# cmhungsteve/TA3N

Hardware: AMD Instinct MI355X
Metric: src+tgt videos/sec per train step, UCF->HMDB_full 5-seg TA3N (higher is better)
Workload: dtype bf16

## Files before the change

### ta3n_amd/csrc/ta3n_gemm_kernel.h

```cpp
#pragma once
#include <hip/hip_runtime.h>
#include <cstdlib>
#include <cstring>

#include <type_traits>

#include "ta3n_kernels.h"

using namespace ta3n;

namespace {

typedef float f32x16 __attribute__((ext_vector_type(16)));
typedef __attribute__((address_space(3))) void lds_void_t;

constexpr int BKC = 64;

__device__ __forceinline__ float4 zero4() { return make_float4(0.f, 0.f, 0.f, 0.f); }

__device__ __forceinline__ void glds16(const float *gsrc, unsigned lds_byte_addr) {
    unsigned keep;
    lds_byte_addr = __builtin_amdgcn_readfirstlane(lds_byte_addr);
    asm volatile("s_mov_b32 %0, m0\n\ts_mov_b32 m0, %2\n\ts_nop 0\n\tglobal_load_lds_dwordx4 %1, off\n\ts_mov_b32 m0, %0"
                 : "=&s"(keep) : "v"(gsrc), "s"(lds_byte_addr) : "memory");
// ... 434 lines not shown
                    unsigned ah[4], al[4], bh[4], bl[4];
#pragma unroll
                    for (int h = 0; h < 2; ++h)
#pragma unroll
                        for (int e = 0; e < 2; ++e) {
                            ah[2 * h + e] = hi2(av[q + h][2 * e], av[q + h][2 * e + 1]);
                            al[2 * h + e] = lo2(av[q + h][2 * e], av[q + h][2 * e + 1], ah[2 * h + e]);
                            bh[2 * h + e] = hi2(bv[q + h][2 * e], bv[q + h][2 * e + 1]);
                            bl[2 * h + e] = lo2(bv[q + h][2 * e], bv[q + h][2 * e + 1], bh[2 * h + e]);
                        }
                    const u32x4 AH = {ah[0], ah[1], ah[2], ah[3]}, AL = {al[0], al[1], al[2], al[3]};
                    const u32x4 BH = {bh[0], bh[1], bh[2], bh[3]}, BL = {bl[0], bl[1], bl[2], bl[3]};
                    acc = __builtin_amdgcn_mfma_f32_32x32x16_bf16(__builtin_bit_cast(bf16x8, AL), __builtin_bit_cast(bf16x8, BH), acc, 0, 0, 0);
                    acc = __builtin_amdgcn_mfma_f32_32x32x16_bf16(__builtin_bit_cast(bf16x8, AH), __builtin_bit_cast(bf16x8, BL), acc, 0, 0, 0);
                    acc = __builtin_amdgcn_mfma_f32_32x32x16_bf16(__builtin_bit_cast(bf16x8, AH), __builtin_bit_cast(bf16x8, BH), acc, 0, 0, 0);
                }
            }
        } else {
#pragma unroll
            for (int q = 0; q < NQ; ++q) {
                if (FULL || 4 * (wk * GPW + 2 * q) < krem) {
                    unsigned ah[2], al[2], bh[2], bl[2];
#pragma unroll
                    for (int e = 0; e < 2; ++e) {
                        ah[e] = hi2(av[q][2 * e], av[q][2 * e + 1]); al[e] = lo2(av[q][2 * e], av[q][2 * e + 1], ah[e]);
                        bh[e] = hi2(bv[q][2 * e], bv[q][2 * e + 1]); bl[e] = lo2(bv[q][2 * e], bv[q][2 * e + 1], bh[e]);
                    }
                    const u32x2 AH = {ah[0], ah[1]}, AL = {al[0], al[1]}, BH = {bh[0], bh[1]}, BL = {bl[0], bl[1]};
                    acc = __builtin_amdgcn_mfma_f32_32x32x8bf16_1k(__builtin_bit_cast(s16x4, AL), __builtin_bit_cast(s16x4, BH), acc, 0, 0, 0);
                    acc = __builtin_amdgcn_mfma_f32_32x32x8bf16_1k(__builtin_bit_cast(s16x4, AH), __builtin_bit_cast(s16x4, BL), acc, 0, 0, 0);
                    acc = __builtin_amdgcn_mfma_f32_32x32x8bf16_1k(__builtin_bit_cast(s16x4, AH), __builtin_bit_cast(s16x4, BH), acc, 0, 0, 0);
                }
            }
        }
        return;
    }
    if (BF) {
        if (NQ % 2 == 0) {
#pragma unroll
            for (int q = 0; q < NQ; q += 2) {
                if (FULL || 4 * (wk * GPW + 2 * q) < krem) {
                    const u32x4 a = {pack_bf16(av[q][0], av[q][1]), pack_bf16(av[q][2], av[q][3]),
                                     pack_bf16(av[q + 1][0], av[q + 1][1]), pack_bf16(av[q + 1][2], av[q + 1][3])};
                    const u32x4 b = {pack_bf16(bv[q][0], bv[q][1]), pack_bf16(bv[q][2], bv[q][3]),
                                     pack_bf16(bv[q + 1][0], bv[q + 1][1]), pack_bf16(bv[q + 1][2], bv[q + 1][3])};
                    acc = __builtin_amdgcn_mfma_f32_32x32x16_bf16(__builtin_bit_cast(bf16x8, a), __builtin_bit_cast(bf16x8, b),
                                                                  acc, 0, 0, 0);
                }
            }
        } else {
#pragma unroll
            for (int q = 0; q < NQ; ++q) {
                if (FULL || 4 * (wk * GPW + 2 * q) < krem) {
                    const u32x2 a = {pack_bf16(av[q][0], av[q][1]), pack_bf16(av[q][2], av[q][3])};
                    const u32x2 b = {pack_bf16(bv[q][0], bv[q][1]), pack_bf16(bv[q][2], bv[q][3])};
                    acc = __builtin_amdgcn_mfma_f32_32x32x8bf16_1k(__builtin_bit_cast(s16x4, a), __builtin_bit_cast(s16x4, b), acc,
                                                                   0, 0, 0);
                }
            }
        }
        return;
    }
#pragma unroll
    for (int q = 0; q < NQ; ++q) {
        if (FULL || 4 * (wk * GPW + 2 * q) < krem) {
#pragma unroll
            for (int j = 0; j < 4; ++j) acc = __builtin_amdgcn_mfma_f32_32x32x2f32(av[q][j], bv[q][j], acc, 0, 0, 0);
        }
    }
}

__device__ __forceinline__ void st_pub(float *p, f32x4 v) { asm volatile("global_store_dwordx4 %0, %1, off sc0 sc1" ::"v"(p), "v"(v) : "memory"); }
__device__ __forceinline__ void st_pub(void *p, u32x2 v) { asm volatile("global_store_dwordx2 %0, %1, off sc0 sc1" ::"v"(p), "v"(v) : "memory"); }
__device__ __forceinline__ void st_pub(float *p, float v) { asm volatile("global_store_dword %0, %1, off sc0 sc1" ::"v"(p), "v"(v) : "memory"); }
__device__ __forceinline__ void st_pub(unsigned short *p, unsigned v) { asm volatile("global_store_short %0, %1, off sc0 sc1" ::"v"(p), "v"(v) : "memory"); }

__device__ __forceinline__ void store_twin4(unsigned short *tp, unsigned w0, unsigned w1, int nrem, bool vec, bool pub) {
    if (nrem >= 4 && vec) {
        if (pub) st_pub(tp, u32x2{w0, w1});
        else *reinterpret_cast<u32x2 *>(tp) = u32x2{w0, w1};
    } else {
        const unsigned short h[4] = {(unsigned short)(w0 & 0xFFFF), (unsigned short)(w0 >> 16), (unsigned short)(w1 & 0xFFFF), (unsigned short)(w1 >> 16)};
#pragma unroll
        for (int e = 0; e < 4; ++e)
            if (e < nrem) { if (pub) st_pub(tp + e, (unsigned)h[e]); else tp[e] = h[e]; }
    }
}

constexpr int CHAIN_SPIN_LIMIT = 1 << 20;
__device__ __forceinline__ void chain_wait(const Task &t, const Wait *__restrict__ waits, int *__restrict__ cnt, int tid, int knobs) {
    const int nwait = (knobs & 1024) ? 0 : t.wait_count;
    if (nwait > 0) {
        if (tid < 64) {
            for (int w0 = 0; w0 < nwait; w0 += 64) {
                const bool mine = w0 + tid < nwait;
                Wait w{0, 0};
                if (mine) w = waits[t.wait_begin + w0 + tid];
                bool ok = !mine;
                int spins = 0;
                for (;;) {
                    if (!ok) ok = ((knobs & 2048) ? __hip_atomic_fetch_add(cnt + 2 + w.counter, 0, __ATOMIC_RELAXED, __HIP_MEMORY_SCOPE_AGENT)
                                                  : __hip_atomic_load(cnt + 2 + w.counter, __ATOMIC_RELAXED, __HIP_MEMORY_SCOPE_AGENT)) >= w.target;
                    if (__all(ok)) break;
                    if (++spins > CHAIN_SPIN_LIMIT) {
                        if (tid == 0) __hip_atomic_store(cnt + 1, 1 + (int)blockIdx.x, __ATOMIC_RELAXED, __HIP_MEMORY_SCOPE_AGENT);
                        break;
                    }
                    if ((spins & 1023) == 0 && __hip_atomic_load(cnt + 1, __ATOMIC_RELAXED, __HIP_MEMORY_SCOPE_AGENT) != 0) break;
                    for (int z = 0; z < (knobs & 255); ++z) __builtin_amdgcn_s_sleep(8);
                }
            }
            if (!(knobs & 256)) __builtin_amdgcn_fence(__ATOMIC_ACQUIRE, "agent");
        }
        __syncthreads();
    }
}
__device__ __forceinline__ void chain_exit(int sig, int *__restrict__ cnt, int n_counters, int tid, int knobs) {
    if ((knobs & 512) && sig < 0) return;
    asm volatile("s_waitcnt vmcnt(0)" ::: "memory");
    __syncthreads();
    if (tid == 0) {
        if (knobs & 512) { __hip_atomic_fetch_add(cnt + 2 + sig, 1, __ATOMIC_RELAXED, __HIP_MEMORY_SCOPE_AGENT); return; }
        if (sig >= 0) {
            const int before = __hip_atomic_fetch_add(cnt + 2 + sig, 1, __ATOMIC_RELAXED, __HIP_MEMORY_SCOPE_AGENT);
            asm volatile("s_waitcnt vmcnt(0)" ::"v"(before) : "memory");
        }
        const int done = __hip_atomic_fetch_add(cnt, 1, __ATOMIC_RELAXED, __HIP_MEMORY_SCOPE_AGENT);
        if (done == (int)gridDim.x - 1) {
            for (int i = 0; i < n_counters; ++i) __hip_atomic_store(cnt + 2 + i, 0, __ATOMIC_RELAXED, __HIP_MEMORY_SCOPE_AGENT);
            __hip_atomic_store(cnt, 0, __ATOMIC_RELAXED, __HIP_MEMORY_SCOPE_AGENT);
        }
    }
}

__device__ __forceinline__ const float *base_ptr(const Ptrs &p, int base) {
    switch (base) {
        case BASE_X: return p.x;
        case BASE_P: return p.p;
        case BASE_G: return p.g;
        case BASE_P16: return p.p16;
        default: return p.ws;
    }
}

}

#ifdef TA3N_GEMM_STAMPS
#define TA3N_STAMP_SLOTS 16
#define TA3N_STAMP_FLOATS (8192 * TA3N_STAMP_SLOTS * 2)
#define GSTAMP_PTR (reinterpret_cast<unsigned long long *>(const_cast<float *>(ptrs.ws) + zeros_off - TA3N_STAMP_FLOATS))
#define GSTAMP(i) do { if (threadIdx.x == 0 && blockIdx.x < 8192) GSTAMP_PTR[blockIdx.x * TA3N_STAMP_SLOTS + (i)] = __builtin_amdgcn_s_memtime(); } while (0)
#define GSTAMP_VAL(i, v) do { if (threadIdx.x == 0 && blockIdx.x < 8192) GSTAMP_PTR[blockIdx.x * TA3N_STAMP_SLOTS + (i)] = (unsigned long long)(v); } while (0)
#define GSTAMP_W1(i, v) do { if (threadIdx.x == 64 && blockIdx.x < 8192) GSTAMP_PTR[blockIdx.x * TA3N_STAMP_SLOTS + (i)] = (unsigned long long)(v); } while (0)
#define KSTAMP_DECL unsigned long long ks_wait = 0, ks_comp = 0, ks_t = 0; int ks_n = 0
#define KSTAMP_BEGIN_WAIT do { ks_t = __builtin_amdgcn_s_memtime(); } while (0)
#define KSTAMP_END_WAIT do { const unsigned long long n_ = __builtin_amdgcn_s_memtime(); ks_wait += n_ - ks_t; ks_t = n_; ++ks_n; } while (0)
#define KSTAMP_END_COMP do { if (ks_t != 0) { const unsigned long long n_ = __builtin_amdgcn_s_memtime(); ks_comp += n_ - ks_t; } } while (0)
#else
#define GSTAMP(i) do { } while (0)
#define GSTAMP_VAL(i, v) do { } while (0)
#define KSTAMP_DECL do { } while (0)
#define KSTAMP_BEGIN_WAIT do { } while (0)
#define KSTAMP_END_WAIT do { } while (0)
#define KSTAMP_END_COMP do { } while (0)
#endif

namespace ta3n {

template <int WM, int WN, int WK, int BF, int NS, int RM, int RN, int KV = 63>
__device__ __forceinline__ void gemm_tile(const Task &t, const Seg *__restrict__ segs, const Ptrs &ptrs, int hyper_off, int zeros_off,
                                          int twin_off, const SgdSide &side, int pair_delta, int knobs) {
    constexpr int NW = WM * WN * WK, NT = 64 * NW;
    constexpr int BM = 32 * WM * RM, BN = 32 * WN * RN;
    constexpr bool HS = BF == 5;
    constexpr int ROWF = HS ? BKC / 2 : BKC;
    constexpr int STAGE = (BM + BN) * ROWF;
    constexpr int CH = BF == 2 ? 2 * BKC : BKC;
    constexpr bool TW = BF == 2 || BF == 4 || BF == 5;
    constexpr bool PAIR = BF == 4;
    constexpr int EPI = NW * RM * RN * 32 * 36;
    constexpr int LDS_FLOATS = NS * STAGE > EPI + 4 ? NS * STAGE : EPI + 4;
    __shared__ __attribute__((aligned(16))) float lds[LDS_FLOATS];

    const int tid = threadIdx.x, lane = tid & 63;
    const int wave = __builtin_amdgcn_readfirstlane(tid >> 6);
    const unsigned lds_base = __builtin_amdgcn_readfirstlane((unsigned)(uintptr_t)(lds_void_t *)lds);
    const int li = lane & 31, lh = lane >> 5;
    const int wk = wave % WK, wn = (wave / WK) % WN, wm = wave / (WK * WN);

    GSTAMP(0);
    constexpr bool OPT = TA3N_EXPERIMENTS != 0 && (KV & 32) != 0;
    const bool pub = OPT && t.sig >= 0 && !(side.p16_off == -12345);
    if (t.epi & EPI_SGD) {
        if (side.params == nullptr) return;
        float part = 0.f;
        if (tid < 256)
            part = strided_partial_sum(ptrs.ws + side.norm_off, side.norm_n, tid, 256);
        part = wave_allreduce_sum(part);
        if (lane == 0 && wave < 4) lds[wave] = part;
        __syncthreads();
        const float total = sqrtf(((lds[0] + lds[1]) + lds[2]) + lds[3]);
        const float coef = clip_coef(total, side.clip);
        float4 *__restrict__ p4 = reinterpret_cast<float4 *>(side.params);
        float4 *__restrict__ m4 = reinterpret_cast<float4 *>(side.momentum);
        const float4 *__restrict__ g4 = reinterpret_cast<const float4 *>(ptrs.g);
        for (int i = t.pad[0] + tid; i < t.pad[1]; i += NT) {
            const float4 p = p4[i], m = m4[i], gr = g4[i];
            float gg[4] = {gr.x, gr.y, gr.z, gr.w}, pp[4] = {p.x, p.y, p.z, p.w}, mm[4] = {m.x, m.y, m.z, m.w};
#pragma unroll
            for (int e = 0; e < 4; ++e) nesterov_sgd(pp[e], mm[e], gg[e] * coef, side.lr, side.mu, side.wd);
            if (pub) st_pub(reinterpret_cast<float *>(p4 + i), f32x4{pp[0], pp[1], pp[2], pp[3]});
            else p4[i] = make_float4(pp[0], pp[1], pp[2], pp[3]);
            m4[i] = make_float4(mm[0], mm[1], mm[2], mm[3]);
            if (side.p16_off >= 0) {
                uint2 *tw = reinterpret_cast<uint2 *>(ptrs.ws + side.p16_off) + i;
                const unsigned h0 = pack_bf16(pp[0], pp[1]), h1 = pack_bf16(pp[2], pp[3]);
                if (pub) st_pub(tw, u32x2{h0, h1});
                else *tw = make_uint2(h0, h1);
                if ((BF == 3 || BF == 4) && pair_delta) {
                    const u32x2 l = {pack_bf16_lo(pp[0], pp[1], h0), pack_bf16_lo(pp[2], pp[3], h1)};
                    if (pub) st_pub(tw + pair_delta / 2, l);
                    else tw[pair_delta / 2] = make_uint2(l[0], l[1]);
                }
            }
        }
        return;
    }
    if (t.epi & EPI_COLSUM) {
        float *__restrict__ dst = const_cast<float *>(base_ptr(ptrs, t.c_base)) + (size_t)t.c_off;
        const float *__restrict__ src = ptrs.ws + t.pad[0];
        float sq = 0.f;
        for (int n = t.n0 + tid; n < t.n_valid; n += NT) {
            float v = 0.f;
            const float *__restrict__ col = src + n;
            const int R = t.pad[1];
            const size_t ld = (size_t)t.pad[2];
            int r = 0;
#pragma unroll 1
            for (; r + 8 <= R; r += 8) {
                float x[8];
#pragma unroll
                for (int i = 0; i < 8; ++i) x[i] = col[(size_t)(r + i) * ld];
#pragma unroll
                for (int i = 0; i < 8; ++i) v += x[i];
            }
            for (; r < R; ++r) v += col[(size_t)r * ld];
            dst[n] = v;
            sq = fmaf(v, v, sq);
            if (OPT && side.p_new != nullptr && t.c_base == BASE_G) {
                const size_t pi = (size_t)t.c_off + n;
                float p1 = ptrs.p[pi], mm = side.momentum[pi];
                nesterov_sgd(p1, mm, v, side.lr, side.mu, side.wd);
                side.p_new[pi] = p1; side.momentum[pi] = mm;
                if (side.p16_new != nullptr) reinterpret_cast<unsigned short *>(side.p16_new)[pi] = (unsigned short)(pack_bf16(p1, 0.f) & 0xFFFF);
            }
        }
        if (t.epi & EPI_SUMSQ) {
            sq = wave_allreduce_sum(sq);
            if (lane == 0) lds[wave] = sq;
            __syncthreads();
            if (tid == 0) {
                float tot = 0.f;
                for (int i = 0; i < NW; ++i) tot += lds[i];
                ptrs.ws[t.pad[3]] = tot;
            }
        }
        return;
    }
    if (t.seg_count == 0) return;
    if (t.epi & EPI_SUMROWS8) {
        const float *__restrict__ src = ptrs.ws + t.pad[1];
        float sacc = 0.f;
        for (int r = tid >> 3; r < t.pad[2]; r += NT / 8) sacc += src[r * 8 + (tid & 7)];
        lds[tid] = sacc;
        __syncthreads();
        if (tid < 8) {
            float v = 0.f;
            for (int i = 0; i < NT / 8; ++i) v += lds[i * 8 + tid];
            ptrs.ws[t.pad[0] + tid] = v;
        }
        __syncthreads();
    }
    const Hyper *__restrict__ hy = reinterpret_cast<const Hyper *>(ptrs.ws + hyper_off);
    const float *__restrict__ zeros = ptrs.ws + zeros_off;
    const uint32_t epi = t.epi;
    struct HyperHead { float beta[3], gamma, lr, momentum, weight_decay, clip, p_drop_i, p_drop_v; uint32_t seed_i, seed_v; };
    const HyperHead hh = *reinterpret_cast<const HyperHead *>(hy);
    const int h_train = hy->train;
    auto scale_of = [&](int kind) -> float {
        switch (kind) {
            case SK_NEG_BETA_REL: return -hh.beta[0];
            case SK_NEG_BETA_VID: return -hh.beta[1];
            case SK_NEG_BETA_FRM: return -hh.beta[2];
            case SK_INV_KEEP_I: return (h_train && hh.p_drop_i > 0.f) ? (hh.p_drop_i < 1.f ? 1.f / (1.f - hh.p_drop_i) : 0.f) : 1.f;
            case SK_INV_KEEP_V: return (h_train && hh.p_drop_v > 0.f) ? (hh.p_drop_v < 1.f ? 1.f / (1.f - hh.p_drop_v) : 0.f) : 1.f;
            case SK_REVERSE_MU: return hy->reverse ? -hy->mu : 1.f;
            default: return 1.f;
        }
    };
    float ebias[4] = {0.f, 0.f, 0.f, 0.f};
    if (epi & EPI_BIAS) {
        const float *__restrict__ bias = base_ptr(ptrs, t.bias_base) + t.bias_off;
        const int n = t.n0 + (tid % (BN / 4)) * 4;
#pragma unroll
        for (int e = 0; e < 4; ++e)
            if (n + e < t.n_valid) ebias[e] = bias[n + e];
    }

    constexpr int ITER_E = (BM * BN / 4 + NT - 1) / NT;
    constexpr bool UPD_PREFETCH = ITER_E <= 2;
    const bool upd_early = OPT && UPD_PREFETCH && side.p_new != nullptr && t.c_base == BASE_G;
    float up_e[UPD_PREFETCH ? ITER_E : 1][4], um_e[UPD_PREFETCH ? ITER_E : 1][4];
    if (upd_early) {
        const bool cv = ((t.c_off | t.c_ld) & 3) == 0;
#pragma unroll
        for (int it = 0; it < (UPD_PREFETCH ? ITER_E : 1); ++it) {
            const int idx = tid + it * NT;
            const int mm_ = t.m0 + idx / (BN / 4), nn_ = t.n0 + (idx % (BN / 4)) * 4;
            const int nr_ = (idx < BM * BN / 4 && mm_ < t.m_valid) ? t.n_valid - nn_ : 0;
            const size_t pi = (size_t)t.c_off + (size_t)mm_ * t.c_ld + nn_;
#pragma unroll
            for (int e = 0; e < 4; ++e) { up_e[it][e] = 0.f; um_e[it][e] = 0.f; }
            if (nr_ >= 4 && cv) {
                const float4 q4 = *reinterpret_cast<const float4 *>(ptrs.p + pi), r4 = *reinterpret_cast<const float4 *>(side.momentum + pi);
                up_e[it][0] = q4.x; up_e[it][1] = q4.y; up_e[it][2] = q4.z; up_e[it][3] = q4.w;
                um_e[it][0] = r4.x; um_e[it][1] = r4.y; um_e[it][2] = r4.z; um_e[it][3] = r4.w;
            } else if (nr_ > 0) {
#pragma unroll
                for (int e = 0; e < 4; ++e) if (e < nr_) { up_e[it][e] = ptrs.p[pi + e]; um_e[it][e] = side.momentum[pi + e]; }
            }
        }
    }

    constexpr bool EPI_EARLY = TA3N_EXPERIMENTS == 0 && KV != 63 && KV != 1;
    constexpr int PF_IT = (EPI_EARLY && ITER_E <= 2) ? ITER_E : 0;
    constexpr bool PF_FAN = PF_IT == 1;
    struct EpiOperands { const float *aux, *add; bool aux_vec, add_vec; int nfan; };
    auto epi_operands = [&]() {
        return EpiOperands{(epi & EPI_MASK) ? base_ptr(ptrs, t.aux_base) + t.aux_off : nullptr,
                           (epi & EPI_ADD) ? base_ptr(ptrs, t.add_base) + t.add_off : nullptr,
                           ((t.aux_off | t.aux_ld) & 3) == 0, ((t.add_off | t.add_ld) & 3) == 0, t.fan_count};
    };
    auto epi_fetch4 = [](float (&o)[4], const float *__restrict__ p, int nrem, bool vec) {
        if (nrem >= 4 && vec) { const float4 q4 = *reinterpret_cast<const float4 *>(p); o[0] = q4.x; o[1] = q4.y; o[2] = q4.z; o[3] = q4.w; }
        else {
#pragma unroll
            for (int e = 0; e < 4; ++e) if (e < nrem) o[e] = p[e];
        }
    };
    auto fetch_add_aux = [&](const EpiOperands &eo, float (&av)[4], float (&mv)[4], int m, int n, int nrem) {
        if (eo.add != nullptr && nrem > 0) epi_fetch4(av, eo.add + (size_t)m * t.add_ld + n, nrem, eo.add_vec);
        if (eo.aux != nullptr && nrem > 0) epi_fetch4(mv, eo.aux + (size_t)m * t.aux_ld + n, nrem, eo.aux_vec);
    };
    auto fetch_fan = [&](const EpiOperands &eo, float (&fm)[3][4], int m, int n, int nrem) {
        if (eo.nfan > 0 && nrem > 0) {
            const bool fan_vec = (t.fan_ld & 3) == 0;
#pragma unroll
            for (int f = 0; f < 3; ++f)
                if (f < eo.nfan)
                    epi_fetch4(fm[f], ptrs.ws + (size_t)t.fan_mask_off[f] + (size_t)m * t.fan_ld + n, nrem, fan_vec && (t.fan_mask_off[f] & 3) == 0);
        }
    };
    EpiOperands eo_early{nullptr, nullptr, false, false, 0};
    float add_e[PF_IT > 0 ? PF_IT : 1][4], aux_e[PF_IT > 0 ? PF_IT : 1][4], fan_e[3][4];
    auto request_epilogue_operands = [&]() {
        eo_early = epi_operands();
#pragma unroll
        for (int it = 0; it < PF_IT; ++it) {
            const int idx = tid + it * NT;
            const int mm_ = t.m0 + idx / (BN / 4), nn_ = t.n0 + (idx % (BN / 4)) * 4;
            const int nr_ = (idx < BM * BN / 4 && mm_ < t.m_valid) ? t.n_valid - nn_ : 0;
#pragma unroll
            for (int e = 0; e < 4; ++e) { add_e[it][e] = 0.f; aux_e[it][e] = 1.f; }
            fetch_add_aux(eo_early, add_e[it], aux_e[it], mm_, nn_, nr_);
            if constexpr (PF_FAN) {
#pragma unroll
                for (int f = 0; f < 3; ++f)
#pragma unroll
                    for (int e = 0; e < 4; ++e) fan_e[f][e] = 0.f;
                fetch_fan(eo_early, fan_e, mm_, nn_, nr_);
            }
        }
    };
    static_assert(PF_IT == 0 || NS == 2, "the early requests are issued from the two-stage K loop (every kind-specialised backward kernel has two stages)");

    f32x16 acc[RM][RN];
#pragma unroll
    for (int i = 0; i < RM; ++i)
#pragma unroll
        for (int j = 0; j < RN; ++j)
#pragma unroll
            for (int r = 0; r < 16; ++r) acc[i][j][r] = 0.f;
    GSTAMP(1);

    const int m0 = t.m0, n0 = t.n0, m_valid = t.m_valid, n_valid = t.n_valid;
    const int seg_end = t.seg_begin + t.seg_count;
    int cseg = t.seg_begin;
    const int ra = wm * (32 * RM) + li, rb = wn * (32 * RN) + li;
    float rs[RM];
#pragma unroll
    for (int i = 0; i < RM; ++i) rs[i] = 0.f;
    (void)knobs;
    KSTAMP_DECL;
    constexpr int KVE = BM > 128 ? (KV & (1 | 2 | 32)) : KV;
    auto k_loop = [&](auto akm, auto bkm, auto rsum) {
        constexpr bool AKM = decltype(akm)::value, BKM = decltype(bkm)::value, RS = decltype(rsum)::value;
        if constexpr (NS == 2) {
            OperandStream<BM, NW, TW, PAIR, HS> oa;
            OperandStream<BN, NW, TW, PAIR, HS> ob;
            int klen = 0, scale = SK_ONE;
            Seg nx = t.seg0;
            auto open_seg = [&](int sidx) {
                const Seg sg = nx;
                if (sidx + 1 < seg_end) nx = segs[sidx + 1];
                klen = sg.klen; scale = sg.scale_kind;
                oa.setup(base_ptr(ptrs, sg.a_base) + (size_t)sg.a_off, sg.a_ld, AKM, sg.klen, m0, sg.pad[0] > 0 ? sg.pad[0] : m_valid,
                         wave, lane, pair_delta);
                ob.setup(base_ptr(ptrs, sg.b_base) + (size_t)sg.b_off, sg.b_ld, BKM, sg.klen, n0, n_valid, wave, lane, pair_delta);
            };
            auto issue = [&](int buf, int k0) {
                const unsigned st = lds_base + (unsigned)(buf * STAGE * 4);
                oa.issue(k0, klen - k0, st, wave, lane, zeros);
                ob.issue(k0, klen - k0, st + BM * ROWF * 4, wave, lane, zeros);
            };
            auto stage_ready = [&]() {
                KSTAMP_END_COMP;
                KSTAMP_BEGIN_WAIT;
                asm volatile("s_waitcnt vmcnt(0)" ::: "memory");
                __builtin_amdgcn_s_barrier();
                asm volatile("" ::: "memory");
                KSTAMP_END_WAIT;
            };
            int buf = 0;
            open_seg(cseg);
            issue(0, 0);
            if constexpr (PF_IT > 0) request_epilogue_operands();
            for (;;) {
                const int n_chunks = (klen + CH - 1) / CH;
                for (int c = 0; c < n_chunks - 1; ++c) {
                    stage_ready();
                    const float *sa = lds + buf * STAGE;
                    issue(buf ^ 1, (c + 1) * CH);
                    compute_stage<BM, BN, WK, AKM, BKM, true, RS, BF, RM, RN>(acc, rs, sa, sa + BM * ROWF, ra, rb, wk, lh, CH);
                    buf ^= 1;
                }
                stage_ready();
                const int krem = klen - (n_chunks - 1) * CH, c_scale = scale;
                ++cseg;
                const bool more = cseg < seg_end;
                if (more) {
                    open_seg(cseg);
                    issue(buf ^ 1, 0);
                }
                const float *sa = lds + buf * STAGE;
                compute_stage<BM, BN, WK, AKM, BKM, false, RS, BF, RM, RN>(acc, rs, sa, sa + BM * ROWF, ra, rb, wk, lh, krem);
                if (c_scale != SK_ONE) {
                    const float sc = scale_of(c_scale);
    #pragma unroll
                    for (int i = 0; i < RM; ++i)
    #pragma unroll
                        for (int j = 0; j < RN; ++j)
    #pragma unroll
                            for (int r = 0; r < 16; ++r) acc[i][j][r] *= sc;
                }
                if (cseg >= seg_end) break;
                buf ^= 1;
            }
            } else {
            OperandStream<BM, NW, TW, PAIR, HS> oa;
            OperandStream<BN, NW, TW, PAIR, HS> ob;
            constexpr int LPW = OperandStream<BM, NW, TW, PAIR, HS>::NP + OperandStream<BN, NW, TW, PAIR, HS>::NP;
            int i_seg = cseg, i_chunk = 0, i_nchunks = 0, i_klen = 0, i_buf = 0, ahead = 0;
            Seg nx = t.seg0;
            auto open_issue_seg = [&]() {
                const Seg sg = nx;
                if (i_seg + 1 < seg_end) nx = segs[i_seg + 1];
                i_klen = sg.klen; i_nchunks = (sg.klen + CH - 1) / CH; i_chunk = 0;
                oa.setup(base_ptr(ptrs, sg.a_base) + (size_t)sg.a_off, sg.a_ld, AKM, sg.klen, m0, sg.pad[0] > 0 ? sg.pad[0] : m_valid,
                         wave, lane, pair_delta);
                ob.setup(base_ptr(ptrs, sg.b_base) + (size_t)sg.b_off, sg.b_ld, BKM, sg.klen, n0, n_valid, wave, lane, pair_delta);
            };
            auto issue_one = [&]() {
                const unsigned st = lds_base + (unsigned)(i_buf * STAGE * 4);
                const int k0 = i_chunk * CH;
                oa.issue(k0, i_klen - k0, st, wave, lane, zeros);
                ob.issue(k0, i_klen - k0, st + BM * ROWF * 4, wave, lane, zeros);
                i_buf = (i_buf + 1 == NS) ? 0 : i_buf + 1;
                ++ahead;
                if (++i_chunk == i_nchunks) {
                    if (++i_seg < seg_end) open_issue_seg();
                }
            };
            auto wait_landed = [&](int younger) {
                static_assert((NS - 2) * LPW <= 63, "vmcnt is a 6-bit counter");
                KSTAMP_END_COMP;
                KSTAMP_BEGIN_WAIT;
                if (NS == 2 || younger == 0) asm volatile("s_waitcnt vmcnt(0)" ::: "memory");
                else if (NS == 3 || younger == 1) asm volatile("s_waitcnt vmcnt(%0)" ::"n"(LPW) : "memory");
                else if (NS == 4 || younger == 2) asm volatile("s_waitcnt vmcnt(%0)" ::"n"(2 * LPW) : "memory");
                else if (NS == 5 || younger == 3) asm volatile("s_waitcnt vmcnt(%0)" ::"n"(3 * LPW) : "memory");
                else asm volatile("s_waitcnt vmcnt(%0)" ::"n"(4 * LPW) : "memory");
                __builtin_amdgcn_s_barrier();
                asm volatile("" ::: "memory");
                KSTAMP_END_WAIT;
            };
            open_issue_seg();
    #pragma unroll 1
            for (int sidx = 0; sidx < NS - 1 && i_seg < seg_end; ++sidx) issue_one();

            int c_buf = 0;
            int c_klen_nx = t.seg0.klen, c_scale_nx = t.seg0.scale_kind;
            for (;;) {
                const int klen = c_klen_nx, c_scale = c_scale_nx;
                if (cseg + 1 < seg_end) { c_klen_nx = segs[cseg + 1].klen; c_scale_nx = segs[cseg + 1].scale_kind; }
                const int n_chunks = (klen + CH - 1) / CH;
                int c = 0;
                if (i_seg == cseg) {
                    for (; c + (NS - 1) < n_chunks; ++c) {
                        wait_landed(NS - 2);
                        const unsigned st = lds_base + (unsigned)(i_buf * STAGE * 4);
                        const int k0 = (c + NS - 1) * CH;
                        const float *sa = lds + c_buf * STAGE;
                        oa.issue(k0, klen - k0, st, wave, lane, zeros);
                        ob.issue(k0, klen - k0, st + BM * ROWF * 4, wave, lane, zeros);
                        compute_stage<BM, BN, WK, AKM, BKM, true, RS, BF, RM, RN>(acc, rs, sa, sa + BM * ROWF, ra, rb, wk, lh, CH);
                        i_buf = (i_buf + 1 == NS) ? 0 : i_buf + 1;
                        c_buf = (c_buf + 1 == NS) ? 0 : c_buf + 1;
                    }
                    if (++i_seg < seg_end) open_issue_seg();
                }
    #pragma unroll 1
                for (; c < n_chunks; ++c) {
                    wait_landed(ahead - 1);
                    if (i_seg < seg_end) issue_one();
                    const float *sa = lds + c_buf * STAGE;
                    if (c < n_chunks - 1)
                        compute_stage<BM, BN, WK, AKM, BKM, true, RS, BF, RM, RN>(acc, rs, sa, sa + BM * ROWF, ra, rb, wk, lh, CH);
                    else
                        compute_stage<BM, BN, WK, AKM, BKM, false, RS, BF, RM, RN>(acc, rs, sa, sa + BM * ROWF, ra, rb, wk, lh, klen - c * CH);
                    c_buf = (c_buf + 1 == NS) ? 0 : c_buf + 1;
                    --ahead;
                }
                if (c_scale != SK_ONE) {
                    const float sc = scale_of(c_scale);
    #pragma unroll
                    for (int i = 0; i < RM; ++i)
    #pragma unroll
                        for (int j = 0; j < RN; ++j)
    #pragma unroll
                            for (int r = 0; r < 16; ++r) acc[i][j][r] *= sc;
                }
                if (++cseg >= seg_end) break;
            }
            }
    };
    using T_ = std::true_type;
    using F_ = std::false_type;
    {
        const Seg &s0 = t.seg0;
        switch (s0.a_kmajor * 2 + s0.b_kmajor) {
            case 0: if constexpr (KVE & 1) k_loop(F_{}, F_{}, F_{}); break;
            case 1: if constexpr (KVE & 2) k_loop(F_{}, T_{}, F_{}); break;
            case 2: if constexpr (KVE & 4) k_loop(T_{}, F_{}, F_{}); break;
            default:
                if (t.epi & EPI_ROWSUM_A) { if constexpr (KVE & 16) k_loop(T_{}, T_{}, T_{}); }
                else { if constexpr (KVE & 8) k_loop(T_{}, T_{}, F_{}); }
                break;
        }
    }

    KSTAMP_END_COMP;
    GSTAMP(2);
#ifdef TA3N_GEMM_STAMPS
    GSTAMP_VAL(8, ks_wait); GSTAMP_VAL(9, ks_comp); GSTAMP_VAL(10, ks_n);
#endif
    __syncthreads();
    GSTAMP(3);
#pragma unroll
    for (int i = 0; i < RM; ++i)
#pragma unroll
        for (int j = 0; j < RN; ++j) {
            float *cs = lds + ((wave * RM + i) * RN + j) * (32 * 36);
#pragma unroll
            for (int r = 0; r < 16; ++r) {
                const int row = (r & 3) + 8 * (r >> 2) + 4 * lh;
                cs[row * 36 + li] = acc[i][j][r];
            }
        }
    __syncthreads();
    GSTAMP(4);

    const float *__restrict__ split_other = nullptr;
    if (OPT && (epi & EPI_SPLITK)) {
        int &split_ticket = *reinterpret_cast<int *>(&lds[EPI]);
        const int half = t.pad[2] - 1;
        float *mine = ptrs.ws + t.pad[0] + (size_t)half * (BM * BN);
        constexpr int ITER_S = (BM * BN / 4 + NT - 1) / NT;
#pragma unroll
        for (int it = 0; it < ITER_S; ++it) {
            const int idx = tid + it * NT;
            if (idx < BM * BN / 4) {
                const int r = idx / (BN / 4), c4 = (idx % (BN / 4)) * 4;
                const int br = r >> 5, bc = c4 >> 5;
                const int slot0 = ((((br / RM) * WN + (bc / RN)) * WK) * RM + (br % RM)) * RN + (bc % RN);
                float4 v4 = zero4();
#pragma unroll
                for (int q = 0; q < WK; ++q) {
                    const float4 part = *reinterpret_cast<const float4 *>(&lds[(slot0 + q * RM * RN) * (32 * 36) + (r & 31) * 36 + (c4 & 31)]);
                    v4.x += part.x; v4.y += part.y; v4.z += part.z; v4.w += part.w;
                }
                st_pub(mine + (size_t)r * BN + c4, f32x4{v4.x, v4.y, v4.z, v4.w});
            }
        }
        asm volatile("s_waitcnt vmcnt(0)" ::: "memory");
        __syncthreads();
        int *ticket = reinterpret_cast<int *>(ptrs.ws + t.pad[1]);
        if (tid == 0) split_ticket = __hip_atomic_fetch_add(ticket, 1, __ATOMIC_RELAXED, __HIP_MEMORY_SCOPE_AGENT);
        __syncthreads();
        if (split_ticket == 0) return;
        if (tid == 0) __hip_atomic_store(ticket, 0, __ATOMIC_RELAXED, __HIP_MEMORY_SCOPE_AGENT);
        split_other = ptrs.ws + t.pad[0] + (size_t)(1 - half) * (BM * BN);
    }
    const float alpha = scale_of(t.alpha_kind);
    const float gamma = scale_of(t.gamma_kind);
    const bool drop_on = (epi & (EPI_DROP_I | EPI_DROP_V)) && h_train != 0;
    const uint32_t dseed = (epi & EPI_DROP_I) ? hh.seed_i : hh.seed_v;
    const float dp = (epi & EPI_DROP_I) ? hh.p_drop_i : hh.p_drop_v;
    const uint32_t doff = drop_on ? (uint32_t)t.pad2 : 0u;
    float *__restrict__ cbase = const_cast<float *>(base_ptr(ptrs, t.c_base)) + (size_t)t.c_off;
    const EpiOperands eo = PF_IT > 0 ? eo_early : epi_operands();
    const int nfan = eo.nfan;
    const bool c_vec = ((t.c_off | t.c_ld) & 3) == 0;
    const bool upd = OPT && side.p_new != nullptr && t.c_base == BASE_G;
    float sumsq = 0.f;
    constexpr int ITER = (BM * BN / 4 + NT - 1) / NT;
    constexpr int UNR = ITER <= 4 ? ITER : 2;
#pragma unroll UNR
    for (int it = 0; it < ITER; ++it) {
        const int idx = tid + it * NT;
        if (idx >= BM * BN / 4) break;
        const int r = idx / (BN / 4);
        const int c4 = (idx % (BN / 4)) * 4;
        const int br = r >> 5, bc = c4 >> 5;
        const int slot0 = ((((br / RM) * WN + (bc / RN)) * WK) * RM + (br % RM)) * RN + (bc % RN);
        const int m = m0 + r, n = n0 + c4;
        const bool row_ok = m < m_valid;
        const int nrem = row_ok ? n_valid - n : 0;
        float av[4] = {0.f, 0.f, 0.f, 0.f}, mv[4] = {1.f, 1.f, 1.f, 1.f};
        float fm[3][4] = {{0.f, 0.f, 0.f, 0.f}, {0.f, 0.f, 0.f, 0.f}, {0.f, 0.f, 0.f, 0.f}};
        if constexpr (PF_IT > 0) {
#pragma unroll
            for (int e = 0; e < 4; ++e) { av[e] = add_e[PF_IT > 0 ? it : 0][e]; mv[e] = aux_e[PF_IT > 0 ? it : 0][e]; asm volatile("" : "+v"(mv[e])); }
        } else {
            fetch_add_aux(eo, av, mv, m, n, nrem);
        }
        if constexpr (PF_FAN) {
#pragma unroll
            for (int f = 0; f < 3; ++f)
#pragma unroll
                for (int e = 0; e < 4; ++e) { fm[f][e] = fan_e[f][e]; asm volatile("" : "+v"(fm[f][e])); }
        } else if constexpr (EPI_EARLY) {
            fetch_fan(eo, fm, m, n, nrem);
        }
        float up[4] = {0.f, 0.f, 0.f, 0.f}, um[4] = {0.f, 0.f, 0.f, 0.f};
        if (upd_early) {
#pragma unroll
            for (int e = 0; e < 4; ++e) { up[e] = up_e[UPD_PREFETCH ? it : 0][e]; um[e] = um_e[UPD_PREFETCH ? it : 0][e]; }
        } else if (upd && nrem > 0) {
            const size_t pi = (size_t)t.c_off + (size_t)m * t.c_ld + n;
            if (nrem >= 4 && c_vec) {
                const float4 q4 = *reinterpret_cast<const float4 *>(ptrs.p + pi), r4 = *reinterpret_cast<const float4 *>(side.momentum + pi);
                up[0] = q4.x; up[1] = q4.y; up[2] = q4.z; up[3] = q4.w; um[0] = r4.x; um[1] = r4.y; um[2] = r4.z; um[3] = r4.w;
            } else {
#pragma unroll
                for (int e = 0; e < 4; ++e) if (e < nrem) { up[e] = ptrs.p[pi + e]; um[e] = side.momentum[pi + e]; }
            }
        }
        float other4[4] = {0.f, 0.f, 0.f, 0.f};
        if (split_other != nullptr) {
            const float *op = split_other + (size_t)r * BN + c4;
#pragma unroll
            for (int e = 0; e < 4; ++e) other4[e] = __hip_atomic_load(op + e, __ATOMIC_RELAXED, __HIP_MEMORY_SCOPE_AGENT);
        }
        float4 v4 = zero4();
#pragma unroll
        for (int q = 0; q < WK; ++q) {
            const float4 part = *reinterpret_cast<const float4 *>(&lds[(slot0 + q * RM * RN) * (32 * 36) + (r & 31) * 36 + (c4 & 31)]);
            v4.x += part.x; v4.y += part.y; v4.z += part.z; v4.w += part.w;
        }
        if (split_other != nullptr) { v4.x += other4[0]; v4.y += other4[1]; v4.z += other4[2]; v4.w += other4[3]; }
#ifdef TA3N_GEMM_STAMPS
        if (it == 0) {
            asm volatile("s_waitcnt lgkmcnt(0)" ::: "memory");
            GSTAMP_W1(11, __builtin_amdgcn_s_memtime());
        }
#endif
        float v[4] = {v4.x, v4.y, v4.z, v4.w};
#pragma unroll
        for (int e = 0; e < 4; ++e) {
            float x = (v[e] + ebias[e]) * alpha + av[e];
            if (epi & EPI_RELU) x = fmaxf(x, 0.f);
            x = mv[e] > 0.f ? x : 0.f;
            if (drop_on) x *= keep_mask(dseed, (uint32_t)(m * t.drop_ld + n + e) + doff, dp);
            v[e] = x * gamma;
        }
        if (nrem <= 0) continue;
#pragma unroll
        for (int e = 0; e < 4; ++e)
            if (e < nrem) sumsq = fmaf(v[e], v[e], sumsq);
        float *cp = cbase + (size_t)m * t.c_ld + n;
        if (epi & EPI_TWIN_ONLY) {
        } else if (nrem >= 4 && c_vec) {
            if (pub) st_pub(cp, f32x4{v[0], v[1], v[2], v[3]});
            else *reinterpret_cast<float4 *>(cp) = make_float4(v[0], v[1], v[2], v[3]);
        } else {
#pragma unroll
            for (int e = 0; e < 4; ++e)
                if (e < nrem) { if (pub) st_pub(cp + e, v[e]); else cp[e] = v[e]; }
        }
        if (upd) {
            const size_t pi = (size_t)t.c_off + (size_t)m * t.c_ld + n;
            float pn[4];
#pragma unroll
            for (int e = 0; e < 4; ++e) {
                pn[e] = up[e];
                nesterov_sgd(pn[e], um[e], v[e], side.lr, side.mu, side.wd);
            }
// ... 150 lines not shown
```

Baseline: 2.024 million.

## Add segment-boundary-aware two-stage K loop that prefetches next segment early

Result: faster. 2.050 million (median of 6 runs) (+1.3%).

```diff
diff --git a/ta3n_amd/csrc/ta3n_gemm_kernel.h b/ta3n_amd/csrc/ta3n_gemm_kernel.h
--- a/ta3n_amd/csrc/ta3n_gemm_kernel.h
+++ b/ta3n_amd/csrc/ta3n_gemm_kernel.h
@@ -610,7 +610,10 @@
 #define GSTAMP(i) do { if (threadIdx.x == 0 && blockIdx.x < 8192) GSTAMP_PTR[blockIdx.x * TA3N_STAMP_SLOTS + (i)] = __builtin_amdgcn_s_memtime(); } while (0)
 #define GSTAMP_VAL(i, v) do { if (threadIdx.x == 0 && blockIdx.x < 8192) GSTAMP_PTR[blockIdx.x * TA3N_STAMP_SLOTS + (i)] = (unsigned long long)(v); } while (0)
 #define GSTAMP_W1(i, v) do { if (threadIdx.x == 64 && blockIdx.x < 8192) GSTAMP_PTR[blockIdx.x * TA3N_STAMP_SLOTS + (i)] = (unsigned long long)(v); } while (0)
-#define KSTAMP_DECL unsigned long long ks_wait = 0, ks_comp = 0, ks_t = 0; int ks_n = 0
+#define KSTAMP_DECL unsigned long long ks_wait = 0, ks_comp = 0, ks_t = 0, ks_bnd = 0, ks_int = 0, ks_mfull = 0, ks_mlast = 0, ks_m0 = 0; int ks_n = 0
+#define KSTAMP_ISSUED(acc) do { acc += (__builtin_amdgcn_s_memtime() - ks_t) + (1ull << 40); } while (0)
+#define KSTAMP_COMP_BEGIN do { ks_m0 = __builtin_amdgcn_s_memtime(); } while (0)
+#define KSTAMP_COMP_DONE(acc) do { acc += (__builtin_amdgcn_s_memtime() - ks_m0) + (1ull << 40); } while (0)
 #define KSTAMP_BEGIN_WAIT do { ks_t = __builtin_amdgcn_s_memtime(); } while (0)
 #define KSTAMP_END_WAIT do { const unsigned long long n_ = __builtin_amdgcn_s_memtime(); ks_wait += n_ - ks_t; ks_t = n_; ++ks_n; } while (0)
 #define KSTAMP_END_COMP do { if (ks_t != 0) { const unsigned long long n_ = __builtin_amdgcn_s_memtime(); ks_comp += n_ - ks_t; } } while (0)
@@ -621,6 +624,13 @@
 #define KSTAMP_BEGIN_WAIT do { } while (0)
 #define KSTAMP_END_WAIT do { } while (0)
 #define KSTAMP_END_COMP do { } while (0)
+#define KSTAMP_ISSUED(acc) do { } while (0)
+#define KSTAMP_COMP_BEGIN do { } while (0)
+#define KSTAMP_COMP_DONE(acc) do { } while (0)
+#endif
+
+#ifndef TA3N_SEG_FAST
+#define TA3N_SEG_FAST 1
 #endif
 
 namespace ta3n {
@@ -842,6 +852,8 @@
     };
     static_assert(PF_IT == 0 || NS == 2, "the early requests are issued from the two-stage K loop (every kind-specialised backward kernel has two stages)");
 
+    constexpr bool SEG_EARLY = TA3N_EXPERIMENTS == 0 && KV != 63 && (BF == 2 || BF == 4) && NS == 2 && (TA3N_SEG_FAST) != 0;
+
     f32x16 acc[RM][RN];
 #pragma unroll
     for (int i = 0; i < RM; ++i)
@@ -863,7 +875,105 @@
     constexpr int KVE = BM > 128 ? (KV & (1 | 2 | 32)) : KV;
     auto k_loop = [&](auto akm, auto bkm, auto rsum) {
         constexpr bool AKM = decltype(akm)::value, BKM = decltype(bkm)::value, RS = decltype(rsum)::value;
-        if constexpr (NS == 2) {
+        if constexpr (SEG_EARLY) {
+            OperandStream<BM, NW, TW, PAIR, HS> oa;
+            OperandStream<BN, NW, TW, PAIR, HS> ob;
+            int i_seg = cseg, i_klen = 0, i_scale = SK_ONE, i_nchunks = 0, i_chunk = 0;
+            int p_klen = 0, p_scale = SK_ONE;
+            Seg nx = t.seg0;
+            bool fetch = false;
+            auto fetch_next = [&]() {
+                if (fetch) {
+                    if (i_seg + 1 < seg_end) nx = segs[i_seg + 1];
+                    fetch = false;
+                }
+            };
+            auto open_issue_seg = [&]() {
+                const Seg sg = nx;
+                fetch = true;
+                i_klen = sg.klen; i_scale = sg.scale_kind; i_nchunks = (sg.klen + CH - 1) / CH; i_chunk = 0;
+                oa.setup(base_ptr(ptrs, sg.a_base) + (size_t)sg.a_off, sg.a_ld, AKM, sg.klen, m0, sg.pad[0] > 0 ? sg.pad[0] : m_valid,
+                         wave, lane, pair_delta);
+                ob.setup(base_ptr(ptrs, sg.b_base) + (size_t)sg.b_off, sg.b_ld, BKM, sg.klen, n0, n_valid, wave, lane, pair_delta);
+            };
+            auto issue_one = [&](int buf) {
+                const unsigned st = lds_base + (unsigned)(buf * STAGE * 4);
+                const int k0 = i_chunk * CH;
+                oa.issue(k0, i_klen - k0, st, wave, lane, zeros);
+                ob.issue(k0, i_klen - k0, st + BM * ROWF * 4, wave, lane, zeros);
+            };
+            auto advance = [&]() {
+                if (++i_chunk == i_nchunks) {
+                    p_klen = i_klen; p_scale = i_scale;
+                    if (++i_seg < seg_end) open_issue_seg();
+                }
+            };
+            auto stage_ready = [&]() {
+                KSTAMP_END_COMP;
+                KSTAMP_BEGIN_WAIT;
+                asm volatile("s_waitcnt vmcnt(0)" ::: "memory");
+                __builtin_amdgcn_s_barrier();
+                asm volatile("" ::: "memory");
+                KSTAMP_END_WAIT;
+            };
+            auto scale_acc = [&](int kind) {
+                if (kind != SK_ONE) {
+                    const float sc = scale_of(kind);
+    #pragma unroll
+                    for (int i = 0; i < RM; ++i)
+    #pragma unroll
+                        for (int j = 0; j < RN; ++j)
+    #pragma unroll
+                            for (int r = 0; r < 16; ++r) acc[i][j][r] *= sc;
+                }
+            };
+            int buf = 0;
+            open_issue_seg();
+            fetch_next();
+            issue_one(0);
+            advance();
+            fetch_next();
+            if constexpr (PF_IT > 0) request_epilogue_operands();
+            for (;;) {
+                const int klen = i_seg == cseg ? i_klen : p_klen, c_scale = i_seg == cseg ? i_scale : p_scale;
+                const int n_full = klen / CH, tail = klen - n_full * CH;
+                for (int c = 0; c < n_full; ++c) {
+                    stage_ready();
+                    const float *sa = lds + buf * STAGE;
+                    if (i_seg < seg_end) {
+#ifdef TA3N_GEMM_STAMPS
+                        const bool ks_first = i_chunk == 0;
+#endif
+                        issue_one(buf ^ 1);
+#ifdef TA3N_GEMM_STAMPS
+                        if (ks_first) KSTAMP_ISSUED(ks_bnd); else KSTAMP_ISSUED(ks_int);
+#endif
+                        advance();
+                    }
+                    KSTAMP_COMP_BEGIN;
+                    compute_stage<BM, BN, WK, AKM, BKM, true, RS, BF, RM, RN>(acc, rs, sa, sa + BM * ROWF, ra, rb, wk, lh, CH);
+#ifdef TA3N_GEMM_STAMPS
+                    if (c + 1 < n_full || tail) KSTAMP_COMP_DONE(ks_mfull); else KSTAMP_COMP_DONE(ks_mlast);
+#endif
+                    fetch_next();
+                    buf ^= 1;
+                }
+                if (tail) {
+                    stage_ready();
+                    const float *sa = lds + buf * STAGE;
+                    if (i_seg < seg_end) {
+                        issue_one(buf ^ 1);
+                        KSTAMP_ISSUED(ks_bnd);
+                        advance();
+                    }
+                    compute_stage<BM, BN, WK, AKM, BKM, false, RS, BF, RM, RN>(acc, rs, sa, sa + BM * ROWF, ra, rb, wk, lh, tail);
+                    fetch_next();
+                    buf ^= 1;
+                }
+                scale_acc(c_scale);
+                if (++cseg >= seg_end) break;
+            }
+        } else if constexpr (NS == 2) {
             OperandStream<BM, NW, TW, PAIR, HS> oa;
             OperandStream<BN, NW, TW, PAIR, HS> ob;
             int klen = 0, scale = SK_ONE;
@@ -899,7 +1009,10 @@
                     stage_ready();
                     const float *sa = lds + buf * STAGE;
                     issue(buf ^ 1, (c + 1) * CH);
+                    KSTAMP_ISSUED(ks_int);
+                    KSTAMP_COMP_BEGIN;
                     compute_stage<BM, BN, WK, AKM, BKM, true, RS, BF, RM, RN>(acc, rs, sa, sa + BM * ROWF, ra, rb, wk, lh, CH);
+                    KSTAMP_COMP_DONE(ks_mfull);
                     buf ^= 1;
                 }
                 stage_ready();
@@ -909,9 +1022,12 @@
                 if (more) {
                     open_seg(cseg);
                     issue(buf ^ 1, 0);
+                    KSTAMP_ISSUED(ks_bnd);
                 }
                 const float *sa = lds + buf * STAGE;
+                KSTAMP_COMP_BEGIN;
                 compute_stage<BM, BN, WK, AKM, BKM, false, RS, BF, RM, RN>(acc, rs, sa, sa + BM * ROWF, ra, rb, wk, lh, krem);
+                if (krem == CH) KSTAMP_COMP_DONE(ks_mlast);
                 if (c_scale != SK_ONE) {
                     const float sc = scale_of(c_scale);
     #pragma unroll
@@ -981,7 +1097,10 @@
                         const float *sa = lds + c_buf * STAGE;
                         oa.issue(k0, klen - k0, st, wave, lane, zeros);
                         ob.issue(k0, klen - k0, st + BM * ROWF * 4, wave, lane, zeros);
+                        KSTAMP_ISSUED(ks_int);
+                        KSTAMP_COMP_BEGIN;
                         compute_stage<BM, BN, WK, AKM, BKM, true, RS, BF, RM, RN>(acc, rs, sa, sa + BM * ROWF, ra, rb, wk, lh, CH);
+                        KSTAMP_COMP_DONE(ks_mfull);
                         i_buf = (i_buf + 1 == NS) ? 0 : i_buf + 1;
                         c_buf = (c_buf + 1 == NS) ? 0 : c_buf + 1;
                     }
@@ -990,12 +1109,26 @@
     #pragma unroll 1
                 for (; c < n_chunks; ++c) {
                     wait_landed(ahead - 1);
+#ifdef TA3N_GEMM_STAMPS
+                    const bool ks_first = i_chunk == 0;
+                    const int ks_ahead = ahead;
+#endif
                     if (i_seg < seg_end) issue_one();
+#ifdef TA3N_GEMM_STAMPS
+                    if (ahead == ks_ahead) { }
+                    else if (ks_first) KSTAMP_ISSUED(ks_bnd);
+                    else KSTAMP_ISSUED(ks_int);
+#endif
                     const float *sa = lds + c_buf * STAGE;
+                    KSTAMP_COMP_BEGIN;
                     if (c < n_chunks - 1)
                         compute_stage<BM, BN, WK, AKM, BKM, true, RS, BF, RM, RN>(acc, rs, sa, sa + BM * ROWF, ra, rb, wk, lh, CH);
                     else
                         compute_stage<BM, BN, WK, AKM, BKM, false, RS, BF, RM, RN>(acc, rs, sa, sa + BM * ROWF, ra, rb, wk, lh, klen - c * CH);
+#ifdef TA3N_GEMM_STAMPS
+                    if (c < n_chunks - 1) KSTAMP_COMP_DONE(ks_mfull);
+                    else if (klen - c * CH == CH) KSTAMP_COMP_DONE(ks_mlast);
+#endif
                     c_buf = (c_buf + 1 == NS) ? 0 : c_buf + 1;
                     --ahead;
                 }
@@ -1031,6 +1164,7 @@
     GSTAMP(2);
 #ifdef TA3N_GEMM_STAMPS
     GSTAMP_VAL(8, ks_wait); GSTAMP_VAL(9, ks_comp); GSTAMP_VAL(10, ks_n);
+    GSTAMP_VAL(12, ks_bnd); GSTAMP_VAL(13, ks_int); GSTAMP_VAL(14, ks_mfull); GSTAMP_VAL(15, ks_mlast);
 #endif
     __syncthreads();
     GSTAMP(3);
```
